# lucanest/Phyloformer

Hardware: AMD Instinct MI355X
Metric: alignments/sec, 60-leaf/500-site LG+GC-like MSAs, Phyloformer forward (pf.ckpt) (higher is better)
Workload: dtype f16x3-split MFMA (two fp16 limbs per operand, 3 passes), fp32 accumulate/residual

## Files before the change

### phyloformer_amd/csrc/pf_device.hip.h

```cpp
#pragma once
#include <hip/hip_runtime.h>
#include <stdint.h>

#include "pf_layout.h"

namespace pfk {

typedef float f32x4 __attribute__((ext_vector_type(4)));
typedef float f32x16 __attribute__((ext_vector_type(16)));
#if PF_F16
typedef _Float16 h16_t;
#define PF_MFMA(a, b, c) __builtin_amdgcn_mfma_f32_32x32x16_f16((a), (b), (c), 0, 0, 0)
#define PF_DOT2C "v_dot2c_f32_f16"
#define PF_CVT_PK "v_cvt_pk_f16_f32"
#define PF_NEG1_LO 0x0000bc00u
#define PF_NEG1_HI 0xbc000000u
#else
typedef __bf16 h16_t;
#define PF_MFMA(a, b, c) __builtin_amdgcn_mfma_f32_32x32x16_bf16((a), (b), (c), 0, 0, 0)
#define PF_DOT2C "v_dot2c_f32_bf16"
#define PF_CVT_PK "v_cvt_pk_bf16_f32"
#define PF_NEG1_LO 0x0000bf80u
#define PF_NEG1_HI 0xbf800000u
#endif
// ... 245 lines not shown
    const float v = (v4[0] + v4[1]) + (v4[2] + v4[3]);
    const float rstd = __builtin_amdgcn_rsqf(pair_sum(v) * (1.f / 64.f) + LN_EPS);
#pragma unroll
    for (int j = 0; j < 32; ++j) xn[j] *= rstd;
}

typedef const f32x4 __attribute__((address_space(3)))* lds_f32x4_t;
__device__ __forceinline__ void load_acc_bias(f32x16& acc, lds_f32_t lds_bias_h) {
#pragma unroll
    for (int q4 = 0; q4 < 4; ++q4) {
        const f32x4 bb = *(lds_f32x4_t)(lds_bias_h + 8 * q4);
#pragma unroll
        for (int i = 0; i < 4; ++i) acc[4 * q4 + i] = bb[i];
    }
}

__device__ __forceinline__ void load_acc_bias(f32x16& acc, const float* lds_bias, int h) {
#pragma unroll
    for (int q4 = 0; q4 < 4; ++q4) {
        const f32x4 bb = *reinterpret_cast<const f32x4*>(lds_bias + 8 * q4 + 4 * h);
#pragma unroll
        for (int i = 0; i < 4; ++i) acc[4 * q4 + i] = bb[i];
    }
}

__device__ __forceinline__ frag_t zero_frag() {
    frag_t z;
#pragma unroll
    for (int i = 0; i < 8; ++i) z[i] = (h16_t)0.f;
    return z;
}

#ifndef PF_DEVICE_HELPERS_ONLY
struct MainArgs {
    float* x;
    float* qrow;
    const float* qcol;
    const frag_t* mfrag;
    const float* rq;
    const float* ctx;
    float* spart;
    float* outpart;
    const frag_t* wimg;
    const float* consts;
    const frag_t* wv_lo;
    const float* table;
    const uint8_t* idx;
    const int16_t* pair_i;
    const int16_t* pair_j;
    int B, N, P, Lloc;
    int flat;
    int nt_aln;
    int slots_aln;
    size_t trash_tok;
    int store_x_last;
    unsigned long long* prof;
    int ablate;
    float* sitemap;
    const float* w;
};

enum { MODE_FIRST = 0, MODE_MID = 1, MODE_LAST = 2, MODE_MID0 = 3, MODE_LAST_FOLD = 4 };

struct TilePos { int b, kt, r0, l0; };
template <bool FLAT>
__device__ __forceinline__ TilePos tile_pos(const MainArgs& a, int task, int ntiles) {
    TilePos q;
    q.b = task / a.nt_aln;
    q.kt = task - q.b * a.nt_aln;
    if (FLAT) { const int tok0 = q.kt * 32; q.r0 = tok0 / a.Lloc; q.l0 = tok0 - q.r0 * a.Lloc; }
    else { q.r0 = q.kt / ntiles; q.l0 = (q.kt - q.r0 * ntiles) * 32; }
    return q;
}
template <bool FLAT>
__device__ __forceinline__ TilePos tile_next(const MainArgs& a, TilePos q) {
    if (++q.kt == a.nt_aln) { q.b++; q.kt = 0; q.r0 = 0; q.l0 = 0; return q; }
    q.l0 += 32;
    if (q.l0 >= a.Lloc) { q.l0 = FLAT ? q.l0 - a.Lloc : 0; q.r0++; }
    return q;
}
struct LanePos { size_t tok0; int toff, l, nvalid, wrap; bool valid, in_r1; };
template <bool FLAT>
__device__ __forceinline__ LanePos lane_pos(const MainArgs& a, const TilePos& q, int t) {
    LanePos o;
    o.tok0 = ((size_t)q.b * a.P + q.r0) * a.Lloc + q.l0;
    const int left = FLAT ? a.P * a.Lloc - q.kt * 32 : a.Lloc - q.l0;
    o.nvalid = min(32, left);
    o.wrap = (FLAT && q.r0 + 1 < a.P) ? min(32, a.Lloc - q.l0) : 32;
    o.valid = t < o.nvalid;
    o.toff = min(t, o.nvalid - 1);
    o.in_r1 = o.toff >= o.wrap;
    o.l = q.l0 + o.toff - (o.in_r1 ? a.Lloc : 0);
    return o;
}
__device__ __forceinline__ void part_range(int flat, int pr, int nparts, int P, int L, int slots_aln, long* first, int* count) {
    if (!flat) { *first = (long)pr * nparts; *count = nparts; return; }
    const int b = pr / P, p = pr - b * P;
    const int k0 = (int)(((long)p * L) >> 5), k1 = (int)((((long)p + 1) * L - 1) >> 5);
    *first = (long)b * slots_aln + k0 + p;
    *count = k1 - k0 + 1;
}

template <int LO, int HI>
__device__ __forceinline__ void image_to_lds(const frag_t* src, unsigned char* smem) {
    static_assert(LO % 64 == 0 && HI % 64 == 0, "the image is copied in whole waves");
    const int wv = threadIdx.x >> 6, ln = threadIdx.x & 63;
#pragma unroll
    for (int k = 0; k < (HI - LO + MAIN_THREADS - 1) / MAIN_THREADS; ++k) {
        const int f0 = LO + k * MAIN_THREADS + wv * 64;
        if (f0 < HI) __builtin_amdgcn_global_load_lds(src + f0 + ln, smem + (size_t)f0 * 16, 16, 0, 0);
    }
}

template <int MODE, bool FLAT, bool SITEMAP = false, bool WEIGHTED = false>
__global__ void __launch_bounds__(MAIN_THREADS, MAIN_WAVES / 4) k_main(MainArgs a) {
    constexpr bool LAST = MODE == MODE_LAST || MODE == MODE_LAST_FOLD;
    constexpr bool FOLD = MODE == MODE_LAST_FOLD;
    static_assert(!SITEMAP || LAST, "the site map is the head's: last block only");
    static_assert(!WEIGHTED || (!SITEMAP && MODE != MODE_FIRST), "weighted launches: blocks' own modes, no site map");
    extern __shared__ __attribute__((aligned(16))) unsigned char smem[];
    lds_frag_t lw = (lds_frag_t)smem;
    lds_f32_t lc = (lds_f32_t)(smem + FRAG_END * 16);

    {
        const float cv = a.consts[min((int)threadIdx.x, CONST_LEN - 1)];
        if (FOLD) {
            image_to_lds<FRAG_W1, FRAG_W2>(a.wimg, smem);
            image_to_lds<FRAG_WO, FRAG_U + U_FRAGS>(a.wimg, smem);
        } else {
            image_to_lds<(MODE == MODE_FIRST) ? FRAG_WV : 0, LAST ? FRAG_WV : FRAG_END>(a.wimg, smem);
        }
        static_assert(CONST_LEN <= MAIN_THREADS, "one constant per thread");
        if (threadIdx.x < CONST_LEN) reinterpret_cast<float*>(smem + FRAG_END * 16)[threadIdx.x] = cv;
        asm volatile("s_waitcnt vmcnt(0)" ::: "memory");
    }
    __syncthreads();

    const int lane = threadIdx.x & 63;
    const int wave = __builtin_amdgcn_readfirstlane(threadIdx.x >> 6);
    const int t = lane & 31;
    const int h = lane >> 5;
    const int ntiles = (a.Lloc + 31) >> 5;
    const int ntasks = a.B * a.nt_aln;
    if (wave >= MAIN_WAVES / 2) __builtin_amdgcn_s_setprio(1);
    unsigned long long tacc[6] = {0, 0, 0, 0, 0, 0}, tprev = 0;
#define PF_TICK(k) do { if (a.prof) { const unsigned long long tn_ = __builtin_amdgcn_s_memtime(); tacc[k] += tn_ - tprev; tprev = tn_; } } while (0)
    if (a.prof) tprev = __builtin_amdgcn_s_memtime();
    lds_frag_t w1p = lw + FRAG_W1 + lane;
    lds_frag_t w2p = lw + FRAG_W2 + lane;
    lds_frag_t wop = lw + FRAG_WO + lane;
    lds_frag_t qkp = lw + FRAG_QK + h * 8 + (t & 7);
    lds_f32_t lch = lc + 4 * h;
    PF_OPAQUE(wop); PF_OPAQUE(qkp); PF_OPAQUE(lch);
    lds_frag_t wvp = wop + (FRAG_WV - FRAG_WO);
    lds_f32_t luh = (lds_f32_t)(smem + FRAG_U * 16) + 16 * h;

    {
        const int nwaves = gridDim.x * MAIN_WAVES;
#ifndef PF_RUN_MAX
#define PF_RUN_MAX 8
#endif
        const int run = max(1, min(PF_RUN_MAX, ntasks / (nwaves * 8)));
        int run0 = (blockIdx.x * MAIN_WAVES + wave) * run;
        const int task0 = run0, task1 = ntasks;
        TilePos cur = tile_pos<FLAT>(a, min(task0, ntasks - 1), ntiles);
        int frag_row = -1;
        frag_t mfr[4];
        f32x4 rqv = {0.f, 0.f, 0.f, 0.f};
        f32x4 px[8], pctx[8], pqr, pqc;
        int pri = 0, prj = 0;
        auto prefetch = [&](const TilePos& np) {
            const LanePos nl = lane_pos<FLAT>(a, np, t);
            const int ll = nl.l, pb = np.b;
            const size_t tk = nl.tok0 + nl.toff;
            if (MODE == MODE_MID0) {
                const uint8_t* ib = a.idx + (size_t)pb * a.N * a.Lloc + ll;
                const int pp = np.r0 + (nl.in_r1 ? 1 : 0);
                pri = residue(ib[(size_t)a.pair_i[pp] * a.Lloc]);
                prj = residue(ib[(size_t)a.pair_j[pp] * a.Lloc]);
            } else {
                const f32x4* xp = reinterpret_cast<const f32x4*>(a.x + tk * 64 + 4 * h);
#pragma unroll
                for (int g = 0; g < 8; ++g) px[g] = xp[2 * g];
            }
            pqr = *reinterpret_cast<const f32x4*>(a.qrow + tk * 4);
            pqc = *reinterpret_cast<const f32x4*>(a.qcol + tk * 4);
            if (MODE != MODE_FIRST) {
                int hq = h;
                asm volatile("" : "+v"(hq));
                const f32x4* cp = reinterpret_cast<const f32x4*>(a.ctx + ((size_t)pb * a.Lloc + ll) * 64 + 4 * hq);
#pragma unroll
                for (int g = 0; g < 8; ++g) pctx[g] = cp[2 * g];
            }
        };
        if (MODE != MODE_FIRST && task0 < task1) prefetch(cur);

        for (int task = task0; task < task1;) {
            const int b = cur.b;
            const int row = b * a.P + cur.r0;
            int ntask = task + 1;
            TilePos nxt = tile_next<FLAT>(a, cur);
            if (ntask == run0 + run) {
                run0 += nwaves * run;
                ntask = run0;
                if (ntask < task1) nxt = tile_pos<FLAT>(a, ntask, ntiles);
            }
            const LanePos lp = lane_pos<FLAT>(a, cur, t);
            const bool straddle = lp.wrap < 32;
            int ai = 0, aj = 0;
            if (MODE == MODE_FIRST) { const int pp = cur.r0 + (lp.in_r1 ? 1 : 0); ai = a.pair_i[pp]; aj = a.pair_j[pp]; }
            auto load_mfr = [&](int r) {
                const frag_t* mf = a.mfrag + (size_t)r * 128 + t;
#pragma unroll
                for (int q = 0; q < 4; ++q) mfr[q] = mf[q * 32];
                typedef const f32x4 __attribute__((address_space(4)))* const_f32x4_t;
                rqv = *(const_f32x4_t)(unsigned long long)(a.rq + (size_t)__builtin_amdgcn_readfirstlane(r) * 4);
                frag_row = r;
            };
            if (MODE != MODE_FIRST && row != frag_row) load_mfr(row);
            const bool valid = lp.valid;
            const int lc_ = lp.l;
            const size_t tok = lp.tok0 + lp.toff;
            float x[32];
            float zh[4] = {0.f, 0.f, 0.f, 0.f};
            float wt = 1.f;
            if (WEIGHTED && LAST) wt = a.w[(size_t)b * a.Lloc + lc_];

            if (MODE == MODE_FIRST) {
                const int ri = residue(a.idx[((size_t)b * a.N + ai) * a.Lloc + lc_]);
                const int rj = residue(a.idx[((size_t)b * a.N + aj) * a.Lloc + lc_]);
                const f32x4* ti = reinterpret_cast<const f32x4*>(a.table + ri * 64 + 4 * h);
                const f32x4* tj = reinterpret_cast<const f32x4*>(a.table + rj * 64 + 4 * h);
#pragma unroll
                for (int g = 0; g < 8; ++g) {
                    f32x4 u = ti[2 * g], w = tj[2 * g];
#pragma unroll
                    for (int i = 0; i < 4; ++i) x[4 * g + i] = u[i] + w[i];
                }
            } else {
                if (MODE == MODE_MID0) {
                    const f32x4* ti = reinterpret_cast<const f32x4*>(a.table + pri * 64 + 4 * h);
                    const f32x4* tj = reinterpret_cast<const f32x4*>(a.table + prj * 64 + 4 * h);
#pragma unroll
                    for (int g = 0; g < 8; ++g) {
                        const f32x4 u = ti[2 * g], w = tj[2 * g];
#pragma unroll
                        for (int i = 0; i < 4; ++i) x[4 * g + i] = u[i] + w[i];
                    }
                } else {
#pragma unroll
                    for (int g = 0; g < 8; ++g)
#pragma unroll
                        for (int i = 0; i < 4; ++i) x[4 * g + i] = px[g][i];
                }
                PF_TICK(0);
                if (!(a.ablate & 8)) {
                    f32x16 ya[2];
#pragma unroll
                    for (int j = 0; j < 32; ++j) ya[j >> 4][j & 15] = x[j];
                    {
                        const f32x4 qr = pqr;
                        auto mix = [&](const bool mine) {
                            float v[8];
#pragma unroll
                            for (int i = 0; i < 4; ++i) v[i] = mine ? qr[i] * rqv[i] : 0.f;
                            v[4] = v[5] = mine ? 1.f : 0.f;
                            v[6] = v[7] = 0.f;
                            frag_t qb_hi, qb_lo;
                            split8(v, qb_hi, qb_lo);
#pragma unroll
                            for (int To = 0; To < 2; ++To) mfma3(ya[To], mfr[To * 2], mfr[To * 2 + 1], qb_hi, qb_lo, To == 1);
                        };
                        mix(h == 0 && !lp.in_r1);
                        if (straddle) {
                            load_mfr(row + 1);
                            mix(h == 0 && lp.in_r1);
                        }
                    }
                    {
                        const f32x4 qc = pqc * COLAPPLY_B_SCALE;
                        float o[32];
#pragma unroll
                        for (int g = 0; g < 8; ++g) {
                            const f32x4 u = pctx[g];
#pragma unroll
                            for (int i = 0; i < 4; ++i) o[4 * g + i] = u[i] * qc[g >> 1];
                        }
#pragma unroll
                        for (int s = 0; s < 4; ++s) {
                            frag_t ob_hi, ob_lo;
                            split8(&o[8 * s], ob_hi, ob_lo);
#pragma unroll
                            for (int To = 0; To < 2; ++To) {
                                lds_frag_t f = wop + ((To * 4 + s) * 2) * 64;
                                const frag_t a_hi = f[0], a_lo = f[64];
                                mfma3(ya[To], a_hi, a_lo, ob_hi, ob_lo, To == 1);
                            }
                        }
                    }
#pragma unroll
                    for (int j = 0; j < 32; ++j) x[j] = ya[j >> 4][j & 15];
                }

                PF_TICK(1);
                if (FOLD) {
#pragma unroll
                    for (int g = 0; g < 8; ++g) {
                        const f32x4 w4 = *(lds_f32x4_t)(lch + CONST_HW + 8 * g);
#pragma unroll
                        for (int i = 0; i < 4; ++i) zh[i] = fmaf(w4[i], x[4 * g + i], zh[i]);
                    }
                }
                if (FOLD && !(a.ablate & 16)) {
                    frag_t xb_hi[4], xb_lo[4];
                    {
                        float xn[32];
                        ln_pair(x, xn);
#pragma unroll
                        for (int s = 0; s < 4; ++s) split8(&xn[8 * s], xb_hi[s], xb_lo[s]);
                    }
                    if (ntask < task1) prefetch(nxt);
                    PF_TICK(2);
#pragma unroll 1
                    for (int T = 0; T < 8; ++T) {
                        f32x16 ha;
                        lds_frag_t f1 = w1p + T * 512;
                        lds_f32_t bp = lch + CONST_B1 + 32 * T;
                        lds_f32_t up = luh + 32 * T;
                        PF_OPAQUE(f1); PF_OPAQUE(bp); PF_OPAQUE(up);
                        load_acc_bias(ha, bp);
                        frag_t fh = f1[0], fl = f1[64];
#pragma unroll
                        for (int s = 0; s < 4; ++s) {
                            frag_t nh = fh, nl = fl;
                            if (s < 3) { nh = f1[(s + 1) * 128]; nl = f1[(s + 1) * 128 + 64]; }
                            mfma3(ha, fh, fl, xb_hi[s], xb_lo[s]);
                            fh = nh; fl = nl;
                        }
#pragma unroll
                        for (int q = 0; q < 4; ++q) {
                            const f32x4 u4 = *(lds_f32x4_t)(up + 4 * q);
#pragma unroll
                            for (int i = 0; i < 4; ++i) zh[i] = fmaf(u4[i], gelu_scaled(ha[4 * q + i]), zh[i]);
                        }
                    }
                    PF_TICK(3);
                } else if (!(a.ablate & 16)) {
                    frag_t xb_hi[4], xb_lo[4];
                    {
                        float xn[32];
                        ln_pair(x, xn);
#pragma unroll
                        for (int s = 0; s < 4; ++s) split8(&xn[8 * s], xb_hi[s], xb_lo[s]);
                    }
                    f32x16 oa[2];
                    load_acc_bias(oa[0], lch + CONST_B2);
                    load_acc_bias(oa[1], lch + CONST_B2 + 32);
#pragma unroll
                    for (int j = 0; j < 32; ++j) oa[j >> 4][j & 15] += x[j];
                    if (ntask < task1) prefetch(nxt);
                    PF_TICK(2);
#pragma unroll 1
                    for (int T = 0; T < 8; ++T) {
                        f32x16 ha;
                        lds_frag_t f1 = w1p + T * 512;
                        lds_frag_t f2 = w2p + T * 256;
                        lds_f32_t bp = lch + CONST_B1 + 32 * T;
                        PF_OPAQUE(f1); PF_OPAQUE(f2); PF_OPAQUE(bp);
                        load_acc_bias(ha, bp);
                        frag_t fh = f1[0], fl = f1[64];
#pragma unroll
                        for (int s = 0; s < 4; ++s) {
                            frag_t nh, nl;
                            if (s < 3) { nh = f1[(s + 1) * 128]; nl = f1[(s + 1) * 128 + 64]; }
                            else { nh = f2[0]; nl = f2[64]; }
                            mfma3(ha, fh, fl, xb_hi[s], xb_lo[s]);
                            fh = nh; fl = nl;
                        }
                        frag_t g_hi[2], g_lo[2];
                        gelu_split8(ha, 0, g_hi[0], g_lo[0]);
                        gelu_split8(ha, 8, g_hi[1], g_lo[1]);
#pragma unroll
                        for (int st = 0; st < 4; ++st) {
                            const int u = st >> 1, To = st & 1;
                            frag_t nh = fh, nl = fl;
                            if (st < 3) {
                                const int nu = (st + 1) >> 1, nTo = (st + 1) & 1;
                                nh = f2[(nTo * 32 + nu * 2) * 64];
                                nl = f2[(nTo * 32 + nu * 2) * 64 + 64];
                            }
                            mfma3(oa[To], fh, fl, g_hi[u], g_lo[u], To == 1);
                            fh = nh; fl = nl;
                        }
                    }
                    PF_TICK(3);
#pragma unroll
                    for (int j = 0; j < 32; ++j) x[j] = oa[j >> 4][j & 15];
                }
            }

            if (!LAST && !(a.ablate & 4)) {
                frag_t wl[8];
#pragma unroll
                for (int i = WVLO_LDS; i < 8; ++i) wl[i] = a.wv_lo[i * 64 + lane];
                if (WEIGHTED) wt = a.w[(size_t)b * a.Lloc + lc_];
                __builtin_amdgcn_sched_barrier(0);
                {
                    const size_t stok = valid ? tok : a.trash_tok + t;
                    f32x4* xo = reinterpret_cast<f32x4*>(a.x + stok * 64 + 4 * h);
#pragma unroll
                    for (int g = 0; g < 8; ++g) {
                        f32x4 u = {x[4 * g], x[4 * g + 1], x[4 * g + 2], x[4 * g + 3]};
                        xo[2 * g] = u;
                    }
                }
                if (a.ablate & 32) { cur = nxt; task = ntask; continue; }
                f32x16 va[3];
                {
                    float xn[32];
                    ln_pair(x, xn);
                    frag_t xb_hi[4], xb_lo[4];
#pragma unroll
                    for (int s = 0; s < 4; ++s) split8(&xn[8 * s], xb_hi[s], xb_lo[s]);
#pragma unroll
                    for (int s = 0; s < 4; ++s) {
                        const frag_t q_hi = qkp[(s * 2) * 16], q_lo = qkp[(s * 2 + 1) * 16];
                        if (s == 0) mfma3_zero(va[2], q_hi, q_lo, xb_hi[s], xb_lo[s]);
                        else mfma3(va[2], q_hi, q_lo, xb_hi[s], xb_lo[s]);
                    }
#pragma unroll
                    for (int s = 0; s < 4; ++s)
#pragma unroll
                        for (int T = 0; T < 2; ++T) {
                            const frag_t f_hi = wvp[(T * 4 + s) * 64];
                            const frag_t f_lo = T * 4 + s < WVLO_LDS ? wvp[(FRAG_WVLO - FRAG_WV) + (T * 4 + s) * 64] : wl[T * 4 + s];
                            if (s == 0) mfma3_zero(va[T], f_hi, f_lo, xb_hi[s], xb_lo[s], T == 1);
                            else mfma3(va[T], f_hi, f_lo, xb_hi[s], xb_lo[s], T == 1);
                        }
                }
#pragma unroll
                for (int r = 0; r < 4; ++r) va[2][r] += lc[CONST_BQK + 4 * h + r];
                float qk[4], ot[4];
#pragma unroll
                for (int i = 0; i < 4; ++i) qk[i] = elu1_fast(va[2][i]);
#pragma unroll
                for (int i = 0; i < 4; ++i) ot[i] = pair_other(qk[i], h);
                float qn[4], kn[4];
#pragma unroll
                for (int i = 0; i < 4; ++i) {
                    qn[i] = h ? ot[i] : qk[i];
                    kn[i] = h ? qk[i] : ot[i];
                }
                {
                    const size_t stok = valid ? tok : a.trash_tok + t;
                    f32x4 qs = {qn[0], qn[1], qn[2], qn[3]};
                    *reinterpret_cast<f32x4*>(a.qrow + stok * 4) = qs;
                }
                const long slot0 = (long)b * a.slots_aln + cur.kt + (FLAT ? cur.r0 : 0);
                for (int part = 0; part < (straddle ? 2 : 1); ++part) {
                    float* sp = a.spart + (size_t)(slot0 + part) * SROW;
                    const float vm = (valid && lp.in_r1 == (part == 1)) ? (WEIGHTED ? wt : 1.f) : 0.f;
                    float km[4];
#pragma unroll
                    for (int i = 0; i < 4; ++i) km[i] = kn[i] * vm;
                    {
                        float qk8[8];
#pragma unroll
                        for (int i = 0; i < 4; ++i) { qk8[i] = vm * qn[i]; qk8[4 + i] = km[i]; }
                        const float sqk = treduce8(qk8, t);
                        if (lane < 8) sp[64 + lane] = sqk;
                    }
                    {
                        float kv[32];
#pragma unroll
                        for (int j = 0; j < 32; ++j) kv[j] = km[j >> 3] * va[j >> 4][j & 15];
                        sp[kmap(t, h)] = treduce32(kv, t);
                    }
                }
            } else if (LAST) {
                float z = 0.f;
                if (FOLD) {
                    z = pair_sum((zh[0] + zh[1]) + (zh[2] + zh[3])) + lc[CONST_C0];
                } else {
#pragma unroll
                    for (int g = 0; g < 8; ++g) {
                        const f32x4 w4 = *(lds_f32x4_t)(lch + CONST_HW + 8 * g);
#pragma unroll
                        for (int i = 0; i < 4; ++i) z = fmaf(w4[i], x[4 * g + i], z);
                    }
                    z = pair_sum(z) + lc[CONST_HB];
                }
                const float spz = softplus20(z);
                const long slot0 = (long)b * a.slots_aln + cur.kt + (FLAT ? cur.r0 : 0);
                for (int part = 0; part < (straddle ? 2 : 1); ++part) {
                    const float so = half32_sum((valid && lp.in_r1 == (part == 1)) ? (WEIGHTED ? wt * spz : spz) : 0.f);
                    if (lane == 0) a.outpart[slot0 + part] = so;
                }
                if (SITEMAP && valid && h == 0) a.sitemap[lp.tok0 + lp.toff] = spz;
                if (!FOLD && a.store_x_last && valid) {
                    f32x4* xo = reinterpret_cast<f32x4*>(a.x + tok * 64 + 4 * h);
#pragma unroll
                    for (int g = 0; g < 8; ++g) {
                        f32x4 u = {x[4 * g], x[4 * g + 1], x[4 * g + 2], x[4 * g + 3]};
                        xo[2 * g] = u;
                    }
                }
            }
            PF_TICK(4);
            cur = nxt;
            task = ntask;
        }
    }
    if (a.prof && __builtin_amdgcn_mbcnt_hi(~0u, __builtin_amdgcn_mbcnt_lo(~0u, 0u)) == 0) {
#pragma unroll
        for (int k = 0; k < 6; ++k) atomicAdd(a.prof + k, tacc[k]);
    }
#undef PF_TICK
}

constexpr int EMBED_THREADS = 512;
constexpr int EMBED_LDS_BYTES = (PAIRTAB_ROWS * PAIRTAB_W + 22 * 64) * 4;
struct EmbedArgs {
    const uint8_t* idx;
    const int16_t* pair_i;
    const int16_t* pair_j;
    const float* ptab;
    const float* table;
    float* x;
    float* qrow;
    float* srow;
    int B, N, P, Lloc;
    unsigned* bad_idx;
    const float* w;
};

template <bool WEIGHTED = false>
__global__ void __launch_bounds__(EMBED_THREADS) k_embed(EmbedArgs a) {
    extern __shared__ __attribute__((aligned(16))) float esm[];
    float* tab = esm;
    float* emb = esm + PAIRTAB_ROWS * PAIRTAB_W;
    {
        constexpr int NV = PAIRTAB_ROWS * PAIRTAB_W / 4, FULL = NV / EMBED_THREADS;
        const f32x4* src = reinterpret_cast<const f32x4*>(a.ptab);
        f32x4* dst = reinterpret_cast<f32x4*>(tab);
        const int wv = threadIdx.x >> 6, ln = threadIdx.x & 63;
#pragma unroll
        for (int k = 0; k < FULL; ++k) {
            const int v0 = k * EMBED_THREADS + wv * 64;
            __builtin_amdgcn_global_load_lds(src + v0 + ln, tab + (size_t)v0 * 4, 16, 0, 0);
        }
        const int it = FULL * EMBED_THREADS + threadIdx.x;
        const f32x4 tail = src[min(it, NV - 1)];
        const f32x4* s2 = reinterpret_cast<const f32x4*>(a.table);
        f32x4* d2 = reinterpret_cast<f32x4*>(emb);
        static_assert(22 * 64 / 4 <= EMBED_THREADS, "one embedding vector per thread");
        const f32x4 ev = s2[min((int)threadIdx.x, 22 * 64 / 4 - 1)];
        if (it < NV) dst[it] = tail;
        if (threadIdx.x < 22 * 64 / 4) d2[threadIdx.x] = ev;
        asm volatile("s_waitcnt vmcnt(0)" ::: "memory");
    }
    __syncthreads();
    const int lane = threadIdx.x & 63, wave = threadIdx.x >> 6;
    const int sg = lane >> 4, cl = lane & 15;
// ... 629 lines not shown
```

### phyloformer_amd/csrc/pf_layout.h

```cpp
#pragma once

#ifndef PF_F16
#define PF_F16 1
#endif

namespace pfk {

constexpr int E = 64;
constexpr int NH = 4;
constexpr int HD = 16;
constexpr int FF = 256;
constexpr int NA = 22;
constexpr int SROW = 72;
constexpr int MROW = 4 * 64;
constexpr float LN_EPS = 1e-5f;

constexpr int FRAG_W1 = 0;
constexpr int FRAG_W2 = FRAG_W1 + 8 * 4 * 2 * 64;
constexpr int FRAG_WO = FRAG_W2 + 2 * 16 * 2 * 64;
constexpr int FRAG_WV = FRAG_WO + 2 * 4 * 2 * 64;
constexpr int FRAG_QK = FRAG_WV + 2 * 4 * 64;
#ifndef PF_WVLO_LDS
#define PF_WVLO_LDS 4
#endif
constexpr int WVLO_LDS = PF_WVLO_LDS;
constexpr int FRAG_WVLO = FRAG_QK + 4 * 2 * 16;
constexpr int FRAG_END = FRAG_WVLO + WVLO_LDS * 64;
constexpr int FRAG_U = FRAG_WV;
constexpr int U_FRAGS = FF * 4 / 16;
static_assert(FRAG_U + U_FRAGS <= FRAG_END, "the folded head fits the last block's tail");
constexpr int WVLO_FRAGS = 2 * 4 * 64;
constexpr int CONST_B1 = 0, CONST_B2 = 256, CONST_BQK = 320, CONST_HW = 328, CONST_HB = 392,
              CONST_C0 = 393, CONST_BOC = 400;
constexpr int CONST_LEN = 464;
constexpr int MAIN_LDS_BYTES = FRAG_END * 16 + CONST_LEN * 4;
constexpr int MFRAG_PER_PAIR = 2 * 2 * 32;

constexpr int MAIN_THREADS = 512;
constexpr int MAIN_WAVES = MAIN_THREADS / 64;

constexpr int PAIRTAB_ROWS = 22 * 22, PAIRTAB_W = 72;

}
```

### phyloformer_amd/csrc/pf_lib.hip

```cpp
#include <hip/hip_runtime.h>
#include <dlfcn.h>

#include <algorithm>
#include <cmath>
#include <cstdarg>
#include <cstdio>
#include <cstdlib>
#include <cstring>
#include <functional>
#include <map>
#include <mutex>
#include <string>
#include <type_traits>
#include <vector>

#include "../../include/phyloformer_amd.h"
#include "pf_device.hip.h"
#include "pf_mha.hip.h"
#include "pf_precise.hip.h"
#include "pf_generic.hip.h"
#include "pf_boot.hip.h"
#include "pf_sites.hip.h"
#include "pf_sitemap.hip.h"
#include "pf_sites_host.h"
// ... 111 lines not shown
struct PreciseWeights {
    F64Ends ends;
    double* blob = nullptr;
    std::vector<pfp::AttnW> row, col;
    std::vector<pfp::FfnW> ffn;
};

struct GenericWeights {
    F64Ends ends;
    bool ready = false;
    std::vector<pfg::AttnW> row, col;
    std::vector<pfg::FfnW> ffn;
};

constexpr int64_t SUB_FLOATS_DEFAULT = (int64_t)1 << 22;

struct DeviceBuffer {
    void* p = nullptr; size_t cap = 0;
    explicit DeviceBuffer(std::vector<DeviceBuffer*>& all) { all.push_back(this); }
    DeviceBuffer(const DeviceBuffer&) = delete;
    int reserve(pf_handle* h, size_t bytes);
    void release() { if (p) hipFree(p); p = nullptr; cap = 0; }
};
template <class T> struct Buffer : DeviceBuffer {
    using DeviceBuffer::DeviceBuffer;
    operator T*() const { return static_cast<T*>(p); }
};

}

struct pf_handle {
    int device = 0;
    int n_blocks = 0;
    hipStream_t stream = nullptr;
    hipStream_t stream2 = nullptr;
    hipStream_t cur = nullptr;
    hipEvent_t ev_fork = nullptr, ev_join = nullptr;
    hipDeviceProp_t prop;
    std::string err;
    int64_t max_seqs = 200;
    bool profile = false;
    bool profile_main_only = false;
    bool debug_keep = false;
    int ablate = 0;
    unsigned long long* phase_prof = nullptr;
    bool phase_prof_last = false;
    bool head_fold = true;
    bool force_rccl = false;
    int64_t ws_limit_bytes = (int64_t)24 << 30;
    float* table = nullptr;
    float* pair_table = nullptr;
    bool embed_mfma = false;
    int colstats_fine = -1;
    bool colstats_ring = true;
    bool materialize_x0 = false;
    float* first_consts = nullptr;
    float* first_img = nullptr;
    std::vector<BlockDev> blk;
    std::vector<void*> owned;
    std::vector<DeviceBuffer*> buffers;
    int pair_n = -1;
    Buffer<int16_t> pair_i{buffers}, pair_j{buffers};
    Buffer<char> ws{buffers}, ws2{buffers};
    bool overlap = true;
    int reserve_cus = 8;
    Buffer<uint8_t> d_idx{buffers};
    Buffer<float> d_out{buffers};
    Buffer<uint8_t> d_rep{buffers};
    Buffer<int32_t> d_map{buffers};
    Buffer<float> d_smap{buffers}, d_se{buffers}, d_prof{buffers};
    Buffer<double> d_mpart{buffers};
    Buffer<char> d_sub{buffers};
    int64_t sub_floats = SUB_FLOATS_DEFAULT;
    pftile::Plan tiled_plan;
    pftile::Tables tiled_tab;
    Buffer<char> d_tiled_tab{buffers};
    Buffer<char> d_nj{buffers}, d_nj_io{buffers};
    int64_t nj_calls = 0;
    int64_t bionj_calls = 0;
    Buffer<char> d_bme{buffers};
    Buffer<float> d_bme_preds{buffers};
    int64_t bme_calls = 0;
    int64_t spr_calls = 0;
    bool spr_pairs_simple = false;
    int64_t spr_step_cap = 0;
    Buffer<char> d_sup{buffers}, d_sup_io{buffers};
    Buffer<uint8_t> d_sup_bad{buffers};
    int64_t sup_calls = 0;
    int64_t transfer_calls = 0;
    Buffer<char> d_con{buffers}, d_con_io{buffers};
    int64_t con_calls = 0;
    Buffer<float> d_w{buffers}, d_wst{buffers}, d_wtab{buffers};
    void* comm[2] = {nullptr, nullptr};
    int rank = 0, world = 1;
    int64_t coll_calls = 0;
    bool sharded_call = false;
    bool reducing = false;
    bool two_streams = true;
    std::vector<ProfSlot> pending;
    std::vector<hipEvent_t> free_events;
    int64_t prof_n[K_COUNT] = {0};
    double prof_ms[K_COUNT] = {0};
    std::map<std::string, std::vector<float>> taps;
    int tile_force = -1;
    int precise = -1;
    double recheck_above = 8.0;
// ... 273 lines not shown
hipEvent_t get_event(pf_handle* h) {
    if (!h->free_events.empty()) { hipEvent_t e = h->free_events.back(); h->free_events.pop_back(); return e; }
    hipEvent_t e;
    hipEventCreate(&e);
    return e;
}
struct ProfScope {
    pf_handle* h; int kid; hipEvent_t a{}, b{};
    bool on;
    ProfScope(pf_handle* h_, int kid_) : h(h_), kid(kid_) {
        on = h->profile && (!h->profile_main_only || kid_ == K_MAIN);
        if (on) { a = get_event(h); b = get_event(h); hipEventRecord(a, h->cur); }
    }
    ~ProfScope() {
        if (on) { hipEventRecord(b, h->cur); h->pending.push_back({kid, a, b}); }
    }
};
void drain_profile(pf_handle* h) {
    if (h->pending.empty()) return;
    hipStreamSynchronize(h->stream);
    if (h->stream2) hipStreamSynchronize(h->stream2);
    for (auto& s : h->pending) {
        float ms = 0.f;
        if (hipEventElapsedTime(&ms, s.a, s.b) == hipSuccess) { h->prof_n[s.kid]++; h->prof_ms[s.kid] += ms; }
        h->free_events.push_back(s.a);
        h->free_events.push_back(s.b);
    }
    h->pending.clear();
}

int save_tap(pf_handle* h, const std::string& name, const float* dptr, size_t n) {
    std::vector<float>& v = h->taps[name];
    v.resize(n);
    HIPCHK(h, hipStreamSynchronize(h->cur));
    HIPCHK(h, hipMemcpy(v.data(), dptr, n * sizeof(float), hipMemcpyDeviceToHost));
    return PF_OK;
}

int allreduce(pf_handle* h, void* buf, size_t count, int dtype = NCCL_FLOAT) {
    if (!h->sharded_call) return PF_OK;
    if (h->world <= 1 && !h->comm[0]) return PF_OK;
    if (!h->comm[0]) return fail(h, PF_ESTATE, "sharded forward on %d ranks needs pf_comm_init", h->world);
    ProfScope ps(h, K_ALLREDUCE);
    void* comm = h->comm[(h->cur == h->stream2 && h->stream2) ? 1 : 0];
    ++h->coll_calls;
    int rc = g_rccl.AllReduce(buf, buf, count, dtype, NCCL_SUM, comm, h->cur);
    if (rc != 0)
        return fail(h, PF_ERCCL, "ncclAllReduce failed: %s",
                    g_rccl.GetErrorString ? g_rccl.GetErrorString(rc) : "?");
    return PF_OK;
}

template <int MODE, bool SITEMAP = false, bool WEIGHTED = false>
int launch_main(pf_handle* h, const MainArgs& a, int kid) {
    const long ntasks = (long)a.B * a.nt_aln;
    const int cus = std::max(1, h->prop.multiProcessorCount - (h->reducing ? h->reserve_cus : 0));
    const int grid = (int)std::max<long>(1, std::min<long>(cus, (ntasks + MAIN_WAVES - 1) / MAIN_WAVES));
    ProfScope ps(h, kid);
    if (a.flat) hipLaunchKernelGGL((k_main<MODE, true, SITEMAP, WEIGHTED>), dim3(grid), dim3(MAIN_THREADS), MAIN_LDS_BYTES, h->cur, a);
    else hipLaunchKernelGGL((k_main<MODE, false, SITEMAP, WEIGHTED>), dim3(grid), dim3(MAIN_THREADS), MAIN_LDS_BYTES, h->cur, a);
    HIPCHK(h, hipGetLastError());
    return PF_OK;
}

struct RowStats { const float* p; int nparts; int flat; };
struct ShardRun {
    Workspace w;
    const uint8_t* d_idx;
    float* d_out;
    int B, N, P, Lloc, L_total;
    TilePlan tp;
    hipStream_t stream;
    RowStats rs;
    float* d_smap = nullptr;
    const float* d_w = nullptr;
    const float* d_wst = nullptr;
};

int zero_fill(pf_handle* h, float* p, size_t n) {
    HIPCHK(h, hipMemsetAsync(p, 0, n * sizeof(float), h->cur));
    return PF_OK;
}

MainArgs main_args(pf_handle* h, const ShardRun& r) {
    MainArgs m{};
    m.x = r.w.x; m.qrow = r.w.qrow; m.qcol = r.w.qcol;
    m.mfrag = reinterpret_cast<const frag_t*>(r.w.mfrag); m.rq = r.w.rq; m.ctx = r.w.ctx; m.spart = r.w.spart;
    m.outpart = r.w.outpart; m.table = h->table; m.idx = r.d_idx; m.pair_i = h->pair_i; m.pair_j = h->pair_j;
    m.B = r.B; m.N = r.N; m.P = r.P; m.Lloc = r.Lloc;
    m.flat = r.tp.flat; m.nt_aln = r.tp.nt_aln; m.slots_aln = r.tp.slots_aln;
    m.store_x_last = h->debug_keep ? 1 : 0;
    m.trash_tok = (size_t)r.B * r.P * r.Lloc;
    m.ablate = h->ablate;
    m.prof = h->phase_prof_last ? nullptr : h->phase_prof;
    m.w = r.d_w;
    return m;
}

bool x0_on_the_fly(const pf_handle* h) {
    return !h->materialize_x0 && !h->embed_mfma && h->n_blocks > 1;
}

int phase_first(pf_handle* h, const ShardRun& r) {
    if (!r.Lloc) return zero_fill(h, r.w.srow, (size_t)r.B * r.P * SROW);
    int rc;
    if (h->embed_mfma) {
        MainArgs m = main_args(h, r);
        m.wimg = reinterpret_cast<const frag_t*>(h->first_img); m.consts = h->first_consts;
        m.wv_lo = reinterpret_cast<const frag_t*>(h->blk[0].wv_lo);
        rc = launch_main<MODE_FIRST>(h, m, K_EMBED);
// ... 1537 lines not shown
    const size_t T = (size_t)pfnj::table_len(N), S = (size_t)N - 3, b = (size_t)B, r = (size_t)R;
    try {
        std::vector<int32_t> parent((size_t)pfbme::nodes_of(N)), children((size_t)pfbme::nodes_of(N) * 3);
        for (size_t i = 0; i < b * r; ++i)
            if (!(flag && flag[i]) && !pfbme::tree_of_joins(rep + i * T, N, parent.data(), children.data()))
                return fail(h, PF_EINVAL, "source %zu: replicate %zu is not a join table of N=%d sequences", i / r, i % r, N);
    } catch (const std::bad_alloc&) { return fail(h, PF_ENOMEM, "out of host memory for the tables of N=%d sequences", N); }
    HIPCHK(h, hipSetDevice(h->device));
    ++h->con_calls;
    pfcon::Staging io{};
    auto list = [&](auto& v) { pfcon::staging_arrays(v, io, b, r, N, lengths != nullptr); };
    if ((rc2 = h->d_con_io.reserve(h, pfspan::measure(list)))) return rc2;
    pfspan::carve(h->d_con_io, list);
    HIPCHK(h, hipMemcpyAsync(io.rep, rep, b * r * T * sizeof(int32_t), hipMemcpyHostToDevice, h->stream));
    if (lengths) HIPCHK(h, hipMemcpyAsync(io.lengths, lengths, b * r * T * sizeof(double), hipMemcpyHostToDevice, h->stream));
    if (flag) HIPCHK(h, hipMemcpyAsync(io.flag, flag, b * r, hipMemcpyHostToDevice, h->stream));
    const ConsensusOut d{io.n_splits, io.count, io.size, io.parent, io.split_length, io.leaf_parent, io.leaf_length, io.status};
    if ((rc2 = consensus_launch(h, io.rep, lengths ? io.lengths : nullptr, flag ? io.flag : nullptr, B, R, N, percent, nb, d))) return rc2;
    HIPCHK(h, hipMemcpyAsync(o.n_splits, io.n_splits, b * sizeof(int32_t), hipMemcpyDeviceToHost, h->stream));
    HIPCHK(h, hipMemcpyAsync(o.count, io.count, b * S * sizeof(int32_t), hipMemcpyDeviceToHost, h->stream));
    HIPCHK(h, hipMemcpyAsync(o.size, io.size, b * S * sizeof(int32_t), hipMemcpyDeviceToHost, h->stream));
    HIPCHK(h, hipMemcpyAsync(o.parent, io.parent, b * S * sizeof(int32_t), hipMemcpyDeviceToHost, h->stream));
    HIPCHK(h, hipMemcpyAsync(o.leaf_parent, io.leaf_parent, b * (size_t)N * sizeof(int32_t), hipMemcpyDeviceToHost, h->stream));
    if (lengths) {
        HIPCHK(h, hipMemcpyAsync(o.split_length, io.split_length, b * S * sizeof(double), hipMemcpyDeviceToHost, h->stream));
        HIPCHK(h, hipMemcpyAsync(o.leaf_length, io.leaf_length, b * (size_t)N * sizeof(double), hipMemcpyDeviceToHost, h->stream));
    }
    HIPCHK(h, hipMemcpyAsync(o.status, io.status, b, hipMemcpyDeviceToHost, h->stream));
    HIPCHK(h, hipStreamSynchronize(h->stream));
    return PF_OK;
}

}

extern "C" {

int pf_abi_version(void) { return PF_ABI_VERSION; }

uint64_t pf_blob_len(int32_t n_blocks, int32_t n_heads, int32_t embed_dim) {
    return read_blob(nullptr, n_blocks, embed_dim, n_heads).len;
}

static int open_device(int device, pf_handle** out) {
    int ndev = 0;
    hipError_t e = hipGetDeviceCount(&ndev);
    if (e != hipSuccess || ndev == 0)
        return fail(nullptr, PF_EHIP, "no HIP device available (%s); there is no CPU fallback",
                    e != hipSuccess ? hipGetErrorString(e) : "device count is 0");
    if (device < 0 || device >= ndev) return fail(nullptr, PF_EINVAL, "device %d out of range (have %d)", device, ndev);
    pf_handle* h = new pf_handle();
    if (const char* e = getenv("PF_TWO_STREAMS")) h->two_streams = atoi(e) != 0;
    if (getenv("PF_ROW_TILES")) h->tile_force = 0;
    if (getenv("PF_FLAT_TILES")) h->tile_force = 1;
    if (const char* v = getenv("PF_COLSTATS_RING")) h->colstats_ring = atoi(v) != 0;
    h->device = device;
    int rc = PF_OK;
    do {
        if ((e = hipSetDevice(device)) != hipSuccess) { rc = fail(nullptr, PF_EHIP, "hipSetDevice: %s", hipGetErrorString(e)); break; }
        if ((e = hipGetDeviceProperties(&h->prop, device)) != hipSuccess) { rc = fail(nullptr, PF_EHIP, "hipGetDeviceProperties: %s", hipGetErrorString(e)); break; }
        if (std::string(h->prop.gcnArchName).rfind("gfx950", 0) != 0) {
            rc = fail(nullptr, PF_EHIP, "device %d is %s; this library is built for gfx950 only", device, h->prop.gcnArchName);
            break;
        }
        if ((e = hipStreamCreateWithFlags(&h->stream, hipStreamNonBlocking)) != hipSuccess) { rc = fail(nullptr, PF_EHIP, "hipStreamCreate: %s", hipGetErrorString(e)); break; }
        h->cur = h->stream;
        if ((e = hipHostMalloc((void**)&h->bad_idx_host, 3 * sizeof(unsigned), hipHostMallocMapped | hipHostMallocCoherent)) != hipSuccess ||
            (e = hipHostGetDevicePointer((void**)&h->bad_idx_dev, h->bad_idx_host, 0)) != hipSuccess) {
            rc = fail(nullptr, PF_EHIP, "hipHostMalloc (residue flag): %s", hipGetErrorString(e));
            break;
        }
        h->bad_idx_host[0] = h->bad_idx_host[1] = h->bad_idx_host[2] = 0u;
        const struct { const void* fn; int bytes; } big_lds[] = {
            {reinterpret_cast<const void*>(&k_main<MODE_FIRST, false>), MAIN_LDS_BYTES},
            {reinterpret_cast<const void*>(&k_main<MODE_MID, false>), MAIN_LDS_BYTES},
            {reinterpret_cast<const void*>(&k_main<MODE_MID0, false>), MAIN_LDS_BYTES},
            {reinterpret_cast<const void*>(&k_main<MODE_LAST, false>), MAIN_LDS_BYTES},
            {reinterpret_cast<const void*>(&k_main<MODE_LAST_FOLD, false>), MAIN_LDS_BYTES},
            {reinterpret_cast<const void*>(&k_main<MODE_FIRST, true>), MAIN_LDS_BYTES},
            {reinterpret_cast<const void*>(&k_main<MODE_MID, true>), MAIN_LDS_BYTES},
            {reinterpret_cast<const void*>(&k_main<MODE_MID0, true>), MAIN_LDS_BYTES},
            {reinterpret_cast<const void*>(&k_main<MODE_LAST, true>), MAIN_LDS_BYTES},
            {reinterpret_cast<const void*>(&k_main<MODE_LAST_FOLD, true>), MAIN_LDS_BYTES},
            {reinterpret_cast<const void*>(&k_main<MODE_LAST, false, true>), MAIN_LDS_BYTES},
            {reinterpret_cast<const void*>(&k_main<MODE_LAST_FOLD, false, true>), MAIN_LDS_BYTES},
            {reinterpret_cast<const void*>(&k_main<MODE_LAST, true, true>), MAIN_LDS_BYTES},
            {reinterpret_cast<const void*>(&k_main<MODE_LAST_FOLD, true, true>), MAIN_LDS_BYTES},
            {reinterpret_cast<const void*>(&k_main<MODE_MID, false, false, true>), MAIN_LDS_BYTES},
            {reinterpret_cast<const void*>(&k_main<MODE_MID0, false, false, true>), MAIN_LDS_BYTES},
            {reinterpret_cast<const void*>(&k_main<MODE_LAST, false, false, true>), MAIN_LDS_BYTES},
            {reinterpret_cast<const void*>(&k_main<MODE_LAST_FOLD, false, false, true>), MAIN_LDS_BYTES},
            {reinterpret_cast<const void*>(&k_main<MODE_MID, true, false, true>), MAIN_LDS_BYTES},
            {reinterpret_cast<const void*>(&k_main<MODE_MID0, true, false, true>), MAIN_LDS_BYTES},
            {reinterpret_cast<const void*>(&k_main<MODE_LAST, true, false, true>), MAIN_LDS_BYTES},
            {reinterpret_cast<const void*>(&k_main<MODE_LAST_FOLD, true, false, true>), MAIN_LDS_BYTES},
            {reinterpret_cast<const void*>(&k_embed<false>), EMBED_LDS_BYTES},
            {reinterpret_cast<const void*>(&k_embed<true>), EMBED_LDS_BYTES},
        };
        for (const auto& k : big_lds)
            if ((e = hipFuncSetAttribute(k.fn, hipFuncAttributeMaxDynamicSharedMemorySize, k.bytes)) != hipSuccess) {
                rc = fail(nullptr, PF_EHIP, "hipFuncSetAttribute: %s", hipGetErrorString(e));
                break;
            }
        if (rc) break;
    } while (0);
    if (rc) { pf_destroy(h); return rc; }
    *out = h;
// ... 28 lines not shown
        rc = prepare_weights(h, bv, w->blob_len);
        if (!rc) rc = prepare_precise_weights(h, bv, &h->pw);
        if (!rc) {
            try { h->blob_copy.assign(w->blob, w->blob + w->blob_len); }
            catch (const std::bad_alloc&) { rc = fail(h, PF_ENOMEM, "out of host memory copying the weights"); }
        }
    } else {
        h->arch_generic = true;
        rc = prepare_generic_weights(h, bv);
    }
    if (rc) g_create_error = h->err;
    if (rc) { pf_destroy(h); return rc; }
    *out = h;
    return PF_OK;
}

int pf_destroy(pf_handle_t* h) {
    if (!h) return PF_OK;
    hipSetDevice(h->device);
    if (h->stream) hipStreamSynchronize(h->stream);
    if (h->stream2) hipStreamSynchronize(h->stream2);
    for (void*& c : h->comm) if (c && g_rccl.CommDestroy) { g_rccl.CommDestroy(c); c = nullptr; }
    for (auto& s : h->pending) { hipEventDestroy(s.a); hipEventDestroy(s.b); }
    for (auto e : h->free_events) hipEventDestroy(e);
    for (void* p : h->owned) hipFree(p);
    for (DeviceBuffer* b : h->buffers) b->release();
    if (h->stream2) hipStreamDestroy(h->stream2);
    if (h->ev_fork) hipEventDestroy(h->ev_fork);
    if (h->ev_join) hipEventDestroy(h->ev_join);
    if (h->stream) hipStreamDestroy(h->stream);
    if (h->bad_idx_host) hipHostFree(h->bad_idx_host);
    delete h;
    return PF_OK;
}

const char* pf_last_error(const pf_handle_t* h) { return h ? h->err.c_str() : g_create_error.c_str(); }

int pf_set_option(pf_handle_t* h, const char* key, int64_t value) {
    if (!h || !key) return PF_EINVAL;
    const std::string k(key);
    if (k == "max_seqs") h->max_seqs = value;
    else if (k == "profile") { drain_profile(h); h->profile = value != 0; h->profile_main_only = value == 2; }
    else if (k == "debug_keep") h->debug_keep = value != 0;
    else if (k == "embed_mfma") h->embed_mfma = value != 0;
    else if (k == "colstats_fine") h->colstats_fine = value < 0 ? -1 : (value != 0);
    else if (k == "materialize_x0") h->materialize_x0 = value != 0;
    else if (k == "overlap") h->overlap = value != 0;
    else if (k == "two_streams") h->two_streams = value != 0;
    else if (k == "reserve_cus") h->reserve_cus = (int)std::max<int64_t>(0, std::min<int64_t>(value, 128));
    else if (k == "ablate") h->ablate = (int)value;
    else if (k == "head_fold") h->head_fold = value != 0;
    else if (k == "force_rccl") h->force_rccl = value != 0;
    else if (k == "colstats_ring") h->colstats_ring = value != 0;
    else if (k == "precise") h->precise = value < 0 ? -1 : (value != 0);
    else if (k == "recheck_above") h->recheck_above = value > 0 ? (double)value : 0.0;
    else if (k == "precise_ffn_valu") h->precise_ffn_valu = value != 0;
    else if (k == "generic") {
        if (h->arch_generic && !value)
            return fail(h, PF_EINVAL, "embed_dim %d / n_heads %d runs on the generic kernels only (option generic cannot be 0)",
                        h->garch.E, h->garch.NH);
        h->generic = value != 0;
    }
    else if (k == "phase_prof") {
        if (value && !h->phase_prof) { HIPCHK(h, hipMalloc((void**)&h->phase_prof, 64)); h->owned.push_back(h->phase_prof); }
        if (h->phase_prof) HIPCHK(h, hipMemset(h->phase_prof, 0, 64));
        if (!value) h->phase_prof = nullptr;
        h->phase_prof_last = value == 2;
    }
    else if (k == "ws_limit_mb") h->ws_limit_bytes = value << 20;
    else if (k == "spr_pairs_simple") h->spr_pairs_simple = value != 0;
    else if (k == "spr_step_cap") h->spr_step_cap = value > 0 ? value : 0;
    else if (k == "sub_floats") h->sub_floats = value > 0 ? value : SUB_FLOATS_DEFAULT;
    else return fail(h, PF_EINVAL, "unknown option '%s'", key);
    return PF_OK;
}

int pf_forward(pf_handle_t* h, const uint8_t* idx, int32_t B, int32_t N, int32_t L, float* out) {
    if (!h) return PF_EINVAL;
    return forward_host_impl(h, idx, B, N, 0, L, L, out);
}

int pf_resample_sites_device(pf_handle_t* h, const uint8_t* d_src, int32_t B, int32_t N, int32_t L, int32_t r_begin, int32_t R,
                             uint64_t seed, uint8_t* d_dst) {
    if (!h) return PF_EINVAL;
    if (!d_src || !d_dst) return fail(h, PF_EINVAL, "null buffer");
    if (B < 1 || N < 1 || L < 1 || R < 1 || r_begin < 0)
        return fail(h, PF_EINVAL, "bad dimensions B=%d N=%d L=%d r_begin=%d R=%d", B, N, L, r_begin, R);
    size_t n = 0;
    if (!mul_size((size_t)B, (size_t)R, (size_t)N * L, &n))
        return fail(h, PF_EINVAL, "B=%d x R=%d replicates of %d x %d overflow the address space", B, R, N, L);
    HIPCHK(h, hipSetDevice(h->device));
    return launch_resample(h, d_src, B, N, L, r_begin, R, seed, d_dst);
}

int pf_bootstrap(pf_handle_t* h, const uint8_t* idx, int32_t B, int32_t N, int32_t L, int32_t R, uint64_t seed, float* out) {
    if (!h) return PF_EINVAL;
    return bootstrap_impl(h, idx, B, N, L, R, seed, out);
}

int pf_window_count(int32_t L, int32_t W, int32_t step) {
    const int n = pfsites::window_count(L, W, step);
    return n < 0 ? PF_EINVAL : n;
}

int pf_window_start(int32_t L, int32_t W, int32_t step, int32_t s) {
    const int st = pfsites::window_start(L, W, step, s);
// ... 689 lines not shown
```

Before: 544.7.

## Deal main-kernel tile runs down columns to reuse site context across rows

Reworks the per-wave task schedule in the main kernel so each run of tiles steps down a column (same site range, successive pair rows) instead of along consecutive tiles. When the next tile shares the batch and site offset, the per-site ctx prefetch is skipped. The row-fragment (mfrag/rq) load moves into the prefetch so it overlaps compute. The trade is less ctx traffic against reloading row fragments on every tile, and a host-side deal computation selectable by env/option.

```diff
diff --git a/phyloformer_amd/csrc/pf_device.hip.h b/phyloformer_amd/csrc/pf_device.hip.h
--- a/phyloformer_amd/csrc/pf_device.hip.h
+++ b/phyloformer_amd/csrc/pf_device.hip.h
@@ -321,6 +321,7 @@
     int flat;
     int nt_aln;
     int slots_aln;
+    MainDeal deal;
     size_t trash_tok;
     int store_x_last;
     unsigned long long* prof;
@@ -333,17 +334,18 @@
 
 struct TilePos { int b, kt, r0, l0; };
 template <bool FLAT>
-__device__ __forceinline__ TilePos tile_pos(const MainArgs& a, int task, int ntiles) {
+__device__ __forceinline__ TilePos tile_pos(const MainArgs& a, int b, int kt, int ntiles) {
     TilePos q;
-    q.b = task / a.nt_aln;
-    q.kt = task - q.b * a.nt_aln;
+    q.b = b;
+    q.kt = kt;
     if (FLAT) { const int tok0 = q.kt * 32; q.r0 = tok0 / a.Lloc; q.l0 = tok0 - q.r0 * a.Lloc; }
     else { q.r0 = q.kt / ntiles; q.l0 = (q.kt - q.r0 * ntiles) * 32; }
     return q;
 }
 template <bool FLAT>
-__device__ __forceinline__ TilePos tile_next(const MainArgs& a, TilePos q) {
-    if (++q.kt == a.nt_aln) { q.b++; q.kt = 0; q.r0 = 0; q.l0 = 0; return q; }
+__device__ __forceinline__ TilePos tile_next(const MainArgs& a, TilePos q, bool col) {
+    if (col) { q.kt += a.deal.stride; q.r0 += a.deal.rows; return q; }
+    ++q.kt;
     q.l0 += 32;
     if (q.l0 >= a.Lloc) { q.l0 = FLAT ? q.l0 - a.Lloc : 0; q.r0++; }
     return q;
@@ -410,7 +412,6 @@
     const int t = lane & 31;
     const int h = lane >> 5;
     const int ntiles = (a.Lloc + 31) >> 5;
-    const int ntasks = a.B * a.nt_aln;
     if (wave >= MAIN_WAVES / 2) __builtin_amdgcn_s_setprio(1);
     unsigned long long tacc[6] = {0, 0, 0, 0, 0, 0}, tprev = 0;
 #define PF_TICK(k) do { if (a.prof) { const unsigned long long tn_ = __builtin_amdgcn_s_memtime(); tacc[k] += tn_ - tprev; tprev = tn_; } } while (0)
@@ -426,19 +427,33 @@
 
     {
         const int nwaves = gridDim.x * MAIN_WAVES;
-#ifndef PF_RUN_MAX
-#define PF_RUN_MAX 8
-#endif
-        const int run = max(1, min(PF_RUN_MAX, ntasks / (nwaves * 8)));
-        int run0 = (blockIdx.x * MAIN_WAVES + wave) * run;
-        const int task0 = run0, task1 = ntasks;
-        TilePos cur = tile_pos<FLAT>(a, min(task0, ntasks - 1), ntiles);
+        const int nruns = a.B * a.deal.runs_aln;
+        int runi = blockIdx.x * MAIN_WAVES + wave;
+        int left = 0;
+        bool col = false;
+        auto run_first = [&](int u) {
+            const int ub = u / a.deal.runs_aln;
+            int kt, n;
+            deal_run(a.deal, a.nt_aln, u - ub * a.deal.runs_aln, &kt, &n, &col);
+            left = n - 1;
+            return tile_pos<FLAT>(a, ub, kt, ntiles);
+        };
+        bool more = runi < nruns;
+        TilePos cur = run_first(min(runi, nruns - 1));
         int frag_row = -1;
         frag_t mfr[4];
         f32x4 rqv = {0.f, 0.f, 0.f, 0.f};
+        auto load_mfr = [&](int r) {
+            const frag_t* mf = a.mfrag + (size_t)r * 128 + t;
+#pragma unroll
+            for (int q = 0; q < 4; ++q) mfr[q] = mf[q * 32];
+            typedef const f32x4 __attribute__((address_space(4)))* const_f32x4_t;
+            rqv = *(const_f32x4_t)(unsigned long long)(a.rq + (size_t)__builtin_amdgcn_readfirstlane(r) * 4);
+            frag_row = r;
+        };
         f32x4 px[8], pctx[8], pqr, pqc;
         int pri = 0, prj = 0;
-        auto prefetch = [&](const TilePos& np) {
+        auto prefetch = [&](const TilePos& np, const bool keep_ctx) {
             const LanePos nl = lane_pos<FLAT>(a, np, t);
             const int ll = nl.l, pb = np.b;
             const size_t tk = nl.tok0 + nl.toff;
@@ -455,6 +470,10 @@
             pqr = *reinterpret_cast<const f32x4*>(a.qrow + tk * 4);
             pqc = *reinterpret_cast<const f32x4*>(a.qcol + tk * 4);
             if (MODE != MODE_FIRST) {
+                const int nrow = pb * a.P + np.r0;
+                if (nrow != frag_row) load_mfr(nrow);
+            }
+            if (MODE != MODE_FIRST && !keep_ctx) {
                 int hq = h;
                 asm volatile("" : "+v"(hq));
                 const f32x4* cp = reinterpret_cast<const f32x4*>(a.ctx + ((size_t)pb * a.Lloc + ll) * 64 + 4 * hq);
@@ -462,31 +481,25 @@
                 for (int g = 0; g < 8; ++g) pctx[g] = cp[2 * g];
             }
         };
-        if (MODE != MODE_FIRST && task0 < task1) prefetch(cur);
-
-        for (int task = task0; task < task1;) {
+        if (MODE != MODE_FIRST && more) prefetch(cur, false);
+
+        while (more) {
             const int b = cur.b;
             const int row = b * a.P + cur.r0;
-            int ntask = task + 1;
-            TilePos nxt = tile_next<FLAT>(a, cur);
-            if (ntask == run0 + run) {
-                run0 += nwaves * run;
-                ntask = run0;
-                if (ntask < task1) nxt = tile_pos<FLAT>(a, ntask, ntiles);
-            }
+            TilePos nxt = cur;
+            if (left > 0) {
+                --left;
+                nxt = tile_next<FLAT>(a, cur, col);
+            } else {
+                runi += nwaves;
+                more = runi < nruns;
+                if (more) nxt = run_first(runi);
+            }
+            const bool keep_ctx = nxt.b == cur.b && nxt.l0 == cur.l0;
             const LanePos lp = lane_pos<FLAT>(a, cur, t);
             const bool straddle = lp.wrap < 32;
             int ai = 0, aj = 0;
             if (MODE == MODE_FIRST) { const int pp = cur.r0 + (lp.in_r1 ? 1 : 0); ai = a.pair_i[pp]; aj = a.pair_j[pp]; }
-            auto load_mfr = [&](int r) {
-                const frag_t* mf = a.mfrag + (size_t)r * 128 + t;
-#pragma unroll
-                for (int q = 0; q < 4; ++q) mfr[q] = mf[q * 32];
-                typedef const f32x4 __attribute__((address_space(4)))* const_f32x4_t;
-                rqv = *(const_f32x4_t)(unsigned long long)(a.rq + (size_t)__builtin_amdgcn_readfirstlane(r) * 4);
-                frag_row = r;
-            };
-            if (MODE != MODE_FIRST && row != frag_row) load_mfr(row);
             const bool valid = lp.valid;
             const int lc_ = lp.l;
             const size_t tok = lp.tok0 + lp.toff;
@@ -588,7 +601,7 @@
 #pragma unroll
                         for (int s = 0; s < 4; ++s) split8(&xn[8 * s], xb_hi[s], xb_lo[s]);
                     }
-                    if (ntask < task1) prefetch(nxt);
+                    if (more) prefetch(nxt, keep_ctx);
                     PF_TICK(2);
 #pragma unroll 1
                     for (int T = 0; T < 8; ++T) {
@@ -627,7 +640,7 @@
                     load_acc_bias(oa[1], lch + CONST_B2 + 32);
 #pragma unroll
                     for (int j = 0; j < 32; ++j) oa[j >> 4][j & 15] += x[j];
-                    if (ntask < task1) prefetch(nxt);
+                    if (more) prefetch(nxt, keep_ctx);
                     PF_TICK(2);
 #pragma unroll 1
                     for (int T = 0; T < 8; ++T) {
@@ -683,7 +696,7 @@
                         xo[2 * g] = u;
                     }
                 }
-                if (a.ablate & 32) { cur = nxt; task = ntask; continue; }
+                if (a.ablate & 32) { cur = nxt; continue; }
                 f32x16 va[3];
                 {
                     float xn[32];
@@ -777,7 +790,6 @@
             }
             PF_TICK(4);
             cur = nxt;
-            task = ntask;
         }
     }
     if (a.prof && __builtin_amdgcn_mbcnt_hi(~0u, __builtin_amdgcn_mbcnt_lo(~0u, 0u)) == 0) {
diff --git a/phyloformer_amd/csrc/pf_layout.h b/phyloformer_amd/csrc/pf_layout.h
--- a/phyloformer_amd/csrc/pf_layout.h
+++ b/phyloformer_amd/csrc/pf_layout.h
@@ -41,4 +41,44 @@
 
 constexpr int PAIRTAB_ROWS = 22 * 22, PAIRTAB_W = 72;
 
+#if defined(__HIPCC__)
+#define PF_HD __host__ __device__ __forceinline__
+#else
+#define PF_HD inline
+#endif
+
+#ifndef PF_RUN_MAX
+#define PF_RUN_MAX 8
+#endif
+struct MainDeal {
+    int run;
+    int stride;
+    int rows;
+    int col_runs;
+    int runs_aln;
+};
+inline MainDeal main_deal(int flat, int Lloc, int nt_aln, int run, bool column_runs) {
+    MainDeal d{run < 1 ? 1 : run, 0, 0, 0, 0};
+    if (column_runs && d.run >= 2 && Lloc > 0) {
+        int g = 32, r = Lloc % 32;
+        while (r) { const int q = g % r; g = r; r = q; }
+        const int S = flat ? Lloc / g : (Lloc + 31) / 32;
+        const long nsb = nt_aln / ((long)d.run * S);
+        if (nsb > 0) { d.stride = S; d.rows = flat ? 32 / g : 1; d.col_runs = (int)(nsb * S); }
+    }
+    d.runs_aln = d.col_runs + (nt_aln - d.col_runs * d.run + d.run - 1) / d.run;
+    return d;
 }
+PF_HD void deal_run(const MainDeal& d, int nt_aln, int ua, int* kt, int* n, bool* col) {
+    *col = ua < d.col_runs;
+    if (*col) {
+        const int sb = ua / d.stride;
+        *kt = ua + sb * d.stride * (d.run - 1);
+        *n = d.run;
+    } else {
+        *kt = ua * d.run;
+        *n = d.run < nt_aln - *kt ? d.run : nt_aln - *kt;
+    }
+}
+
+}
diff --git a/phyloformer_amd/csrc/pf_lib.hip b/phyloformer_amd/csrc/pf_lib.hip
--- a/phyloformer_amd/csrc/pf_lib.hip
+++ b/phyloformer_amd/csrc/pf_lib.hip
@@ -187,6 +187,7 @@
     float* pair_table = nullptr;
     bool embed_mfma = false;
     int colstats_fine = -1;
+    int column_runs = 1;
     bool colstats_ring = true;
     bool materialize_x0 = false;
     float* first_consts = nullptr;
@@ -566,10 +567,15 @@
 }
 
 template <int MODE, bool SITEMAP = false, bool WEIGHTED = false>
-int launch_main(pf_handle* h, const MainArgs& a, int kid) {
+int launch_main(pf_handle* h, const MainArgs& a0, int kid) {
+    MainArgs a = a0;
     const long ntasks = (long)a.B * a.nt_aln;
     const int cus = std::max(1, h->prop.multiProcessorCount - (h->reducing ? h->reserve_cus : 0));
     const int grid = (int)std::max<long>(1, std::min<long>(cus, (ntasks + MAIN_WAVES - 1) / MAIN_WAVES));
+    const long nwaves = (long)grid * MAIN_WAVES;
+    int run = (int)std::max<long>(1, std::min<long>(PF_RUN_MAX, ntasks / (nwaves * 8)));
+    if (h->column_runs > 1) run = std::min(h->column_runs, PF_RUN_MAX);
+    a.deal = main_deal(a.flat, a.Lloc, a.nt_aln, run, h->column_runs != 0);
     ProfScope ps(h, kid);
     if (a.flat) hipLaunchKernelGGL((k_main<MODE, true, SITEMAP, WEIGHTED>), dim3(grid), dim3(MAIN_THREADS), MAIN_LDS_BYTES, h->cur, a);
     else hipLaunchKernelGGL((k_main<MODE, false, SITEMAP, WEIGHTED>), dim3(grid), dim3(MAIN_THREADS), MAIN_LDS_BYTES, h->cur, a);
@@ -2213,6 +2219,7 @@
     if (const char* e = getenv("PF_TWO_STREAMS")) h->two_streams = atoi(e) != 0;
     if (getenv("PF_ROW_TILES")) h->tile_force = 0;
     if (getenv("PF_FLAT_TILES")) h->tile_force = 1;
+    if (const char* v = getenv("PF_COLUMN_RUNS")) h->column_runs = std::max(0, std::min(atoi(v), PF_RUN_MAX));
     if (const char* v = getenv("PF_COLSTATS_RING")) h->colstats_ring = atoi(v) != 0;
     h->device = device;
     int rc = PF_OK;
@@ -2347,6 +2354,7 @@
     else if (k == "head_fold") h->head_fold = value != 0;
     else if (k == "force_rccl") h->force_rccl = value != 0;
     else if (k == "colstats_ring") h->colstats_ring = value != 0;
+    else if (k == "column_runs") h->column_runs = (int)std::max<int64_t>(0, std::min<int64_t>(value, PF_RUN_MAX));
     else if (k == "precise") h->precise = value < 0 ? -1 : (value != 0);
     else if (k == "recheck_above") h->recheck_above = value > 0 ? (double)value : 0.0;
     else if (k == "precise_ffn_valu") h->precise_ffn_valu = value != 0;
```

Result: no change. 548.5, median of 6 (+0.7%).
